# panbanda/islands

Measured on AMD Instinct MI355X. Metric: queries/sec @ recall@10>=0.95, 10Mx768 ef=128, higher is better.
Workload: dtype f32; 1 GPU; 10000000 x 768 f32 rows resident in HBM (in-memory provider), hierarchical Gaussian mixture, graph by the harness (tools/synth.py::build_graph: k-means medoid levels flattened into one layer, diversified links, parent->child and reverse edges), deg<= 60 (mean 38.6), query batch 1024, k=10, ef=128, cosine; nodes=10000000, dim=768, query_batch=1024, k=10, ef=128, graph=harness, distinct_leaves=False, parallelism=single, searches_in_flight=32, distinct_batches=497, replayed_queries=1688

## Files before the change

### include/islands_amd.h

```cpp
#ifndef ISLANDS_AMD_H
#define ISLANDS_AMD_H

#include <stddef.h>
#include <stdint.h>

#ifdef __cplusplus
extern "C" {
#endif

#define ISL_ABI_VERSION 3

typedef int32_t isl_status;

enum {
  ISL_OK = 0,
  ISL_ERR_DIMENSION_MISMATCH = 1,
  ISL_ERR_EMPTY_COLLECTION = 2,
  ISL_ERR_INVALID_CONFIG = 3,
  ISL_ERR_INDEX_NOT_BUILT = 4,
  ISL_ERR_NODE_NOT_FOUND = 5,
  ISL_ERR_SERIALIZATION = 6,
  ISL_ERR_DESERIALIZATION = 7,
  ISL_ERR_IO = 8,
  ISL_ERR_HNSW = 9,
// ... 150 lines not shown
                                  uint64_t k, uint64_t ef, uint64_t* out_ids, float* out_dist,
                                  uint32_t* out_count, uint64_t* token);
isl_status isl_search_batch_device(const isl_index* idx, const float* d_queries, uint64_t nq,
                                   uint64_t d, uint64_t k, uint64_t ef, uint64_t* d_out_ids,
                                   float* d_out_dist, uint32_t* d_out_count, void* stream);
isl_status isl_search_batch_device_async(const isl_index* idx, const float* d_queries, uint64_t nq,
                                         uint64_t d, uint64_t k, uint64_t ef, uint64_t* d_out_ids,
                                         float* d_out_dist, uint32_t* d_out_count, void* stream,
                                         uint64_t* token);
isl_status isl_search_wait_stats(const isl_index* idx, uint64_t token, isl_search_stats* stats);
isl_status isl_search_wait(const isl_index* idx, uint64_t token);
isl_status isl_search_stream_wait(const isl_index* idx, uint64_t token, void* stream);
isl_status isl_index_group_counters(const isl_index* idx, uint64_t* launches, uint64_t* shared_launches,
                                    uint64_t* shared_calls);
isl_status isl_index_group_markers(const isl_index* idx, uint64_t* calls, uint64_t* marked_calls);
isl_status isl_search(const isl_index* idx, const float* query, uint64_t d, uint64_t k,
                      uint64_t* out_ids, float* out_dist, uint32_t* out_count);

isl_status isl_search_last_stats(const isl_index* idx, isl_search_stats* out);

#define ISL_MAX_ENTRY_SEEDS 65536ull
isl_status isl_index_select_entry_seeds(isl_index* idx, uint64_t count, uint64_t* out_ids, uint64_t* out_count);
isl_status isl_index_set_entry_seeds(isl_index* idx, const uint64_t* ids, uint64_t count);
isl_status isl_index_entry_seeds(const isl_index* idx, uint64_t* out, uint64_t cap, uint64_t* count);
isl_status isl_index_pick_entries(const isl_index* idx, const float* queries, uint64_t nq, uint64_t d,
                                  uint64_t* out_ids, int32_t mem, void* stream);

isl_status isl_distance(int32_t metric, const float* a, uint64_t na, const float* b, uint64_t nb,
                        float* out);
isl_status isl_distance_squared(int32_t metric, const float* a, uint64_t na, const float* b,
// ... 192 lines not shown
```

### include/islands_amd.hpp

```cpp
#pragma once

#include <cstdint>
#include <optional>
#include <stdexcept>
#include <string>
#include <utility>
#include <vector>

#include "islands_amd.h"

namespace islands::core {

struct CoreError : std::runtime_error {
  isl_status status;
  uint64_t expected, actual, node;
  CoreError(isl_status s, const std::string& msg, uint64_t e = 0, uint64_t a = 0, uint64_t n = 0)
      : std::runtime_error(msg), status(s), expected(e), actual(a), node(n) {}
  std::string kind() const { return isl_status_name(status); }
};

inline void check(isl_status s) {
  if (s != ISL_OK)
    throw CoreError(s, isl_last_error_message(), isl_last_error_expected(),
                    isl_last_error_actual(), isl_last_error_node());
// ... 222 lines not shown
    return out;
  }
  void attach_pq_codes(const isl_pq* pq, const std::vector<uint16_t>& codes, uint64_t n) {
    check(isl_index_set_pq_codes(h_, pq, codes.data(), n, ISL_MEM_HOST));
  }
  std::vector<std::pair<uint64_t, float>> search_two_level(const std::vector<float>& query, uint64_t k,
                                                           uint64_t ef, float rerank_ratio) const {
    std::vector<uint64_t> ids(k ? k : 1);
    std::vector<float> dist(k ? k : 1);
    uint32_t cnt = 0;
    check(isl_search_two_level_batch(h_, query.data(), 1, query.size(), k, ef, rerank_ratio, ids.data(),
                                     dist.data(), &cnt));
    std::vector<std::pair<uint64_t, float>> out;
    for (uint32_t i = 0; i < cnt; i++) out.emplace_back(ids[i], dist[i]);
    return out;
  }
  isl_index* handle() const { return h_; }

 private:
  explicit LeannIndex(std::nullptr_t) {}
  isl_index* h_ = nullptr;
};

struct SearchResult {
  uint64_t id = 0;
  float score = 0.f;
  std::optional<std::vector<float>> vector;
  std::optional<std::string> text;
  float to_similarity() const { return 1.0f / (1.0f + score); }
};
// ... 251 lines not shown
```

### islands_amd/_ffi.py

```python
from __future__ import annotations

import ctypes as C
import os

os.environ.setdefault("GPU_MAX_HW_QUEUES", "32")

_HERE = os.path.dirname(os.path.abspath(__file__))
LIB_PATH = os.environ.get("ISL_AMD_LIB") or os.path.join(_HERE, "lib", "libislands_amd.so")

u64, u32, i32, f32 = C.c_uint64, C.c_uint32, C.c_int32, C.c_float
P = C.POINTER


class LeannConfigC(C.Structure):
    _fields_ = [
        ("m", u64), ("m0", u64), ("ef_construction", u64), ("ml", C.c_double),
        ("max_layers", u64), ("metric", u32), ("ef_search", u64), ("beam_width", u64),
        ("prune_ratio", f32), ("pruning_strategy", u32), ("high_degree_pruning", C.c_uint8),
        ("hub_percentile", f32), ("is_compact", C.c_uint8), ("is_recompute", C.c_uint8),
    ]


class BertConfigC(C.Structure):
    _fields_ = [("vocab_size", u32), ("hidden", u32), ("layers", u32), ("heads", u32),
# ... 67 lines not shown
                                         C.c_void_p, C.c_void_p, C.c_void_p]),
    "isl_search_two_level_batch_device": (i32, [C.c_void_p, C.c_void_p, u64, u64, u64, u64,
                                                C.c_float, C.c_void_p, C.c_void_p, C.c_void_p,
                                                C.c_void_p]),
    "isl_search_two_level_batch_device_async": (i32, [C.c_void_p, C.c_void_p, u64, u64, u64, u64,
                                                      C.c_float, C.c_void_p, C.c_void_p, C.c_void_p,
                                                      C.c_void_p, P(u64)]),
    "isl_search_batch_device": (i32, [C.c_void_p, C.c_void_p, u64, u64, u64, u64, C.c_void_p,
                                      C.c_void_p, C.c_void_p, C.c_void_p]),
    "isl_search_batch_device_async": (i32, [C.c_void_p, C.c_void_p, u64, u64, u64, u64, C.c_void_p,
                                            C.c_void_p, C.c_void_p, C.c_void_p, P(u64)]),
    "isl_search_wait": (i32, [C.c_void_p, u64]),
    "isl_search_stream_wait": (i32, [C.c_void_p, u64, C.c_void_p]),
    "isl_index_group_counters": (i32, [C.c_void_p, P(u64), P(u64), P(u64)]),
    "isl_index_group_markers": (i32, [C.c_void_p, P(u64), P(u64)]),
    "isl_shard_record_bytes": (u64, [u64, u64]),
    "isl_merge_topk_packed_async": (i32, [u64, u64, u64, C.c_void_p, u64, C.c_void_p, u64, C.c_void_p, C.c_void_p,
                                          C.c_void_p, C.c_void_p, C.c_void_p, i32, C.c_void_p]),
    "isl_shard_unique_id": (i32, [C.c_void_p]),
    "isl_shard_group_create": (i32, [i32, i32, i32, C.c_void_p, P(C.c_void_p)]),
    "isl_shard_group_create_host": (i32, [i32, i32, i32, C.c_void_p, C.c_void_p, P(C.c_void_p)]),
    "isl_shard_group_info": (i32, [C.c_void_p, P(i32), P(i32), P(i32), P(i32)]),
    "isl_shard_group_free": (None, [C.c_void_p]),
    "isl_sharded_searcher_new": (i32, [C.c_void_p, C.c_void_p, u64, C.c_void_p, i32, P(C.c_void_p)]),
    "isl_sharded_searcher_free": (None, [C.c_void_p]),
    "isl_sharded_prepare": (i32, [C.c_void_p, u64, u64, u64]),
    "isl_sharded_submit": (i32, [C.c_void_p, C.c_void_p, u64, u64, u64, u64, C.c_void_p, P(u64)]),
    "isl_sharded_result": (i32, [C.c_void_p, u64, P(C.c_void_p), P(C.c_void_p), P(C.c_void_p), P(C.c_void_p),
                                 P(SearchStatsC)]),
    "isl_sharded_search_batch": (i32, [C.c_void_p, C.c_void_p, u64, u64, u64, u64, C.c_void_p, C.c_void_p,
# ... 125 lines not shown
```

### islands_amd/csrc/api_index.hip

```cpp
#include "device_common.hip.h"
#include "encoder.hpp"

#include <algorithm>
#include <cmath>
#include <new>

namespace isl {

ErrorRecord& last_error() {
  thread_local ErrorRecord rec;
  return rec;
}

isl_status fail(isl_status st, const char* fmt, ...) {
  char buf[512];
  va_list ap;
  va_start(ap, fmt);
  vsnprintf(buf, sizeof(buf), fmt, ap);
  va_end(ap);
  last_error().message = buf;
  return st;
}

isl_status fail_dim(uint64_t expected, uint64_t actual) {
// ... 38 lines not shown
    g_devices[device].ncu = prop.multiProcessorCount;
    g_devices[device].state = 1;
  }
  return ISL_OK;
}

int device_cu_count(int32_t device) {
  return (device >= 0 && device < 64 && g_devices[device].state == 1) ? g_devices[device].ncu : 256;
}

void free_workspace(SearchWorkspace& ws) {
  if (ws.ev0) (void)hipEventDestroy(ws.ev0);
  if (ws.ev1) (void)hipEventDestroy(ws.ev1);
  if (ws.ev_in) (void)hipEventDestroy(ws.ev_in);
  if (ws.ev_done) (void)hipEventDestroy(ws.ev_done);
  ws = SearchWorkspace{};
}

}

using namespace isl;

static int g_hw_queues_at_load = 4;
__attribute__((constructor)) static void isl_default_hw_queues() {
  if (const char* e = getenv("GPU_MAX_HW_QUEUES")) {
    const int v = atoi(e);
    if (v > 0) g_hw_queues_at_load = v;
  }
  setenv("GPU_MAX_HW_QUEUES", "32", 0);
}
// ... 754 lines not shown
```

### islands_amd/csrc/common.hpp

```cpp
#pragma once

#include <hip/hip_runtime.h>

#include <algorithm>
#include <cstdarg>
#include <cstdint>
#include <cstdlib>
#include <cstdio>
#include <cstring>
#include <atomic>
#include <chrono>
#include <mutex>
#include <string>
#include <thread>
#include <type_traits>
#include <vector>

#include "../../include/islands_amd.h"
#include "device_buffer.hpp"
#include "row_table.hpp"

namespace isl {

struct ErrorRecord {
// ... 45 lines not shown
  DeviceBuffer<uint32_t> qsel;
  DeviceBuffer<uint32_t> qsel_h;
  DeviceBuffer<uint64_t> plog;
  DeviceBuffer<float> q_stage;
  DeviceBuffer<uint64_t> ids_stage;
  DeviceBuffer<float> dist_stage;
  DeviceBuffer<uint32_t> count_stage;
  PinnedBuffer<float> h_q;
  PinnedBuffer<uint64_t> h_ids;
  PinnedBuffer<float> h_dist;
  PinnedBuffer<uint32_t> h_count;
  hipStream_t stream = nullptr;
  hipEvent_t ev0 = nullptr, ev1 = nullptr, ev_in = nullptr, ev_done = nullptr;
  float launch_ms = 0.0f;
  bool launch_ms_read = false;
  bool busy = false;
  bool waiting = false;
  bool enqueued = false;
  bool ticket_clean = false;
  bool publish_results = false;
  uint64_t token = 0;
  uint64_t nq_inflight = 0, k_inflight = 0;
  uint32_t ef_inflight = 0;
  bool fast_inflight = false;
  hipStream_t st_inflight = nullptr;
  uint64_t* u_ids = nullptr;
  float* u_dist = nullptr;
  uint32_t* u_count = nullptr;
  PinnedBuffer<uint32_t> h_status;
  PinnedBuffer<uint32_t> h_ctr;
// ... 26 lines not shown
  uint64_t alloc_mark = 0;
  isl_search_stats stats{};
  bool grp = false;
  SearchWorkspace* grp_launch = nullptr;
  uint32_t grp_offset = 0;
  hipEvent_t grp_ready = nullptr;
  bool grp_marked = false;
  uint64_t grp_allocs = 0;
  bool grp_failed = false;
  isl_status grp_status = ISL_OK;
  ErrorRecord grp_error;
  int32_t pool_lane = -1;
  bool union_launch = false;
  PinnedBuffer<uint64_t> h_members;
  DeviceBuffer<uint32_t> grp_scratch;
};

constexpr int kSearchLanes = 32;

int hw_queues_at_load();
constexpr int kGroupBelowQueues = 8;
struct GroupSwitches { bool off; uint32_t cap, room; bool mark_always, trace; };
inline GroupSwitches group_switches() {
  auto num = [](const char* name) -> uint32_t {
    const char* e = getenv(name);
    const long long v = e ? atoll(e) : 0;
    return v > 0 ? (uint32_t)std::min<long long>(v, 0x7FFFFFFF) : 0u;
  };
  const char* off = getenv("ISL_NO_GROUP");
  const bool is_off = (off && *off) ? strcmp(off, "0") != 0 : hw_queues_at_load() >= kGroupBelowQueues;
// ... 82 lines not shown

  mutable std::mutex mu;
  mutable std::mutex recompute_mu;
  struct RecJoin {
    std::mutex mu;
    std::mutex leader;
    std::vector<void*> waiting;
  };
  mutable RecJoin rec_join;
  mutable isl::SearchWorkspace ws[isl::kSearchLanes];
  mutable isl::ExactPool pool;
  mutable uint64_t next_token = 1;
  const isl::GroupSwitches group_sw = isl::group_switches();
  mutable std::mutex group_mu;
  mutable isl::GroupState* group = nullptr;
};

struct isl_hnsw {
  isl_index* core = nullptr;
  uint64_t m = 0, m0 = 0, ef_construction = 0;
  uint64_t dim = 0;
  double ml = 0.0;
  uint64_t max_layers = 16;
  int32_t device = 0;
  std::vector<const uint64_t*> layer_off;
  std::vector<const uint32_t*> layer_adj;
  mutable std::mutex host_mu;
  mutable bool host_valid = false;
  mutable std::vector<std::vector<uint64_t>> h_off;
  mutable std::vector<std::vector<uint64_t>> h_adj;
// ... 28 lines not shown
```

### islands_amd/csrc/search.hip

```cpp
#include "search_geometry.hpp"
#include "search_internal.hpp"

#include <cmath>

using namespace isl_lane;

namespace {

__global__ void fill_u32_kernel(uint32_t* p, uint64_t n, uint32_t v) {
  uint64_t i = (uint64_t)blockIdx.x * blockDim.x + threadIdx.x;
  uint64_t stride = (uint64_t)gridDim.x * blockDim.x;
  for (; i < n; i += stride) p[i] = v;
}

struct PublishParams {
  const uint32_t* src[6];
  uint32_t* dst[6];
  uint32_t words[6];
  uint32_t ticket_seg;
};
__global__ void publish_kernel(PublishParams pp) {
  const uint32_t seg = blockIdx.y;
  const uint32_t n = pp.words[seg];
  const uint32_t* __restrict__ src = pp.src[seg];
  uint32_t* __restrict__ dst = pp.dst[seg];
  for (uint32_t i = blockIdx.x * blockDim.x + threadIdx.x; i < n; i += gridDim.x * blockDim.x) {
    dst[i] = src[i];
    if (seg == pp.ticket_seg) const_cast<uint32_t*>(src)[i] = 0u;
  }
}
__global__ void copy_u128_kernel(const uint4* __restrict__ src, uint4* __restrict__ dst, uint64_t n) {
  for (uint64_t i = (uint64_t)blockIdx.x * blockDim.x + threadIdx.x; i < n; i += (uint64_t)gridDim.x * blockDim.x)
    dst[i] = src[i];
}
__global__ void copy_u32_kernel(const uint32_t* __restrict__ src, uint32_t* __restrict__ dst, uint64_t n) {
  for (uint64_t i = (uint64_t)blockIdx.x * blockDim.x + threadIdx.x; i < n; i += (uint64_t)gridDim.x * blockDim.x)
    dst[i] = src[i];
}

__global__ void seed_redo_kernel(const uint32_t* __restrict__ list, uint32_t n, uint32_t* __restrict__ redo,
                                 uint32_t* __restrict__ ticket) {
  for (uint32_t i = threadIdx.x; i < n; i += blockDim.x) redo[i] = list[i];
  if (threadIdx.x == 0) ticket[1] = n;
// ... 22 lines not shown
  return st;
}

}

isl_status isl_lane::ensure_lane_stream(const isl_index* idx, isl::SearchWorkspace& ws) {
  if (ws.stream) return ISL_OK;
  bool created = false;
  hipStream_t st = pool_stream(idx->device, ws.pool_lane >= 0 ? (uint32_t)ws.pool_lane : (uint32_t)(&ws - idx->ws), &created);
  if (!st) return isl::fail(ISL_ERR_DEVICE, "hipStreamCreate failed for a search lane");
  if (created) ws.alloc_events++;
  if (!ws.ev_done) { ISL_HIP(hipEventCreateWithFlags(&ws.ev_done, hipEventDisableTiming)); ws.alloc_events++; }
  if (!ws.ev0) { ISL_HIP(hipEventCreate(&ws.ev0)); ws.alloc_events++; }
  if (!ws.ev1) { ISL_HIP(hipEventCreate(&ws.ev1)); ws.alloc_events++; }
  if (!ws.ev_in) { ISL_HIP(hipEventCreateWithFlags(&ws.ev_in, hipEventDisableTiming)); ws.alloc_events++; }
  if (!ws.ticket) {
    ISL_TRY(ws.ticket.reserve(16, &ws.alloc_events));
    ws.ticket_clean = false;
  }
  ISL_TRY(ws.h_head.reserve(16, &ws.alloc_events));
  ws.stream = st;
  return ISL_OK;
}

void isl_lane::copy_words(const uint32_t* src, uint32_t* dst, uint64_t n, uint32_t grid, uint32_t block, hipStream_t st) {
  hipLaunchKernelGGL(copy_u32_kernel, dim3(grid), dim3(block), 0, st, src, dst, n);
}

isl_status isl_lane::prepare_workspace(const isl_index* idx, isl::SearchWorkspace& ws, uint32_t nq, uint32_t slots,
                                       uint32_t plog_cap) {
// ... 72 lines not shown
}

namespace {

__global__ void pad_rows_kernel(const uint64_t* __restrict__ off, const uint32_t* __restrict__ adj, uint64_t n,
                                uint32_t W, uint32_t* __restrict__ ell, uint32_t* __restrict__ deg) {
  const uint64_t row = (uint64_t)blockIdx.x * 4 + (threadIdx.x >> 6);
  const uint32_t lane = threadIdx.x & 63;
  if (row >= n) return;
  const uint64_t o0 = off[row];
  const uint32_t d = (uint32_t)(off[row + 1] - o0);
  for (uint32_t i = lane; i < W; i += 64) ell[row * W + i] = i < d ? adj[o0 + i] : EMPTY;
  if (lane == 0) deg[row] = d;
}

isl_status publish(isl::SearchWorkspace& ws, uint64_t nq, uint64_t k, hipStream_t st) {
  PublishParams pp{};
  uint32_t n = 0;
  auto seg = [&](const void* src, void* dst, uint64_t words) {
    pp.src[n] = (const uint32_t*)src; pp.dst[n] = (uint32_t*)dst; pp.words[n] = (uint32_t)words; ++n;
  };
  seg(ws.status, ws.h_status, nq);
  seg(ws.ctr, ws.h_ctr, nq * 4);
  pp.ticket_seg = n;
  seg(ws.ticket, ws.h_head, 16);
  if (ws.publish_results) {
    seg(ws.count_stage, ws.h_count, nq);
    if (k) {
      seg(ws.ids_stage, ws.h_ids, nq * k * 2);
      seg(ws.dist_stage, ws.h_dist, nq * k);
    }
  }
  hipLaunchKernelGGL(publish_kernel, dim3(16, n), dim3(256), 0, st, pp);
  ISL_HIP(hipGetLastError());
  ws.ticket_clean = true;
  return ISL_OK;
}


void launch_fast(const isl_launch::FastKernel& k, uint32_t grid, size_t lds, hipStream_t st, const SearchParams& p) {
  switch (k.S) {
    case 1: isl_launch::launch_fast_segments<1>(k, grid, lds, st, &p); break;
    case 2: isl_launch::launch_fast_segments<2>(k, grid, lds, st, &p); break;
    case 4: isl_launch::launch_fast_segments<4>(k, grid, lds, st, &p); break;
    default: isl_launch::launch_fast_segments<8>(k, grid, lds, st, &p); break;
  }
}

isl_status search_enqueue_impl(const isl_index* idx, isl::SearchWorkspace& ws, const SearchCall& c,
                               const RoundPlan& plan, bool warm) {
  const uint64_t nq = c.nq, d = c.d, k = c.k;
  if (nq > 0x7FFFFFFFull) return isl::fail(ISL_ERR_INVALID_ARGUMENT, "too many queries");
// ... 203 lines not shown
      launch_fast(fk, grid, cg.fg.lds, st, p);
      p.qsel_mode = 0;
    } else if (!skip_fast) {
      launch_fast(fk, grid, cg.fg.lds, st, p);
    }
    ISL_HIP(hipGetLastError());
    p.nq = (uint32_t)nq;
  } else if (!warm && !resume) {
    std::vector<uint32_t> all(nq);
    for (uint64_t i = 0; i < nq; i++) all[i] = (uint32_t)i;
    uint32_t head0[4] = {0, (uint32_t)nq, 0, 0};
    ISL_HIP(hipMemcpyAsync(ws.redo, all.data(), nq * 4, hipMemcpyHostToDevice, st));
    ISL_HIP(hipMemcpyAsync(ws.ticket, head0, 16, hipMemcpyHostToDevice, st));
    ISL_HIP(hipStreamSynchronize(st));
  }
  if (!tl) {
    uint32_t grid = (uint32_t)std::min<uint64_t>(nq_grid, idx->pool.slots);
    isl_launch::launch_exact(metric, idx->is_hnsw, grid, cg.exact_lds, st, &p);
    ISL_HIP(hipGetLastError());
  }
  ISL_HIP(hipEventRecord(ws.ev1, st));
  ws.st_inflight = st;
  if (warm) return ISL_OK;

  if (!ws.union_launch) {
    ISL_TRY(publish(ws, nq, k, st));
    ISL_HIP(hipEventRecord(ws.ev_done, st));
  }
  ws.enqueued = true;
  ws.nq_inflight = nq;
  ws.k_inflight = k;
  ws.ef_inflight = ef;
  ws.fast_inflight = use_fast;
  return ISL_OK;
}

struct LastStats { const isl_index* idx = nullptr; isl_search_stats st{}; };
thread_local LastStats tl_last_stats;
void note_last_stats(const isl_index* idx, const isl_search_stats& st) {
  tl_last_stats.idx = idx;
  tl_last_stats.st = st;
}

}

isl_status isl_lane::search_enqueue(const isl_index* idx, isl::SearchWorkspace& ws, const SearchCall& c,
                                      const RoundPlan& plan, bool warm) {
  const isl_status st = search_enqueue_impl(idx, ws, c, plan, warm);
  if (st != ISL_OK) {
    const isl::ErrorRecord keep = isl::last_error();
    hipStream_t s = call_stream(ws, c);
    if (c.mode == StreamMode::USER || s) (void)hipStreamSynchronize(s);
    (void)hipGetLastError();
    ws.ticket_clean = false;
    ws.enqueued = false;
    isl::last_error() = keep;
  }
  return st;
}

isl_status isl_lane::search_finish(const isl_index* idx, isl::SearchWorkspace& ws, uint32_t* misses,
                                     bool defer_statuses) {
  if (!ws.enqueued) return isl::fail(ISL_ERR_INVALID_ARGUMENT, "no search in flight for this token");
  ws.enqueued = false;
  const uint64_t nq = ws.nq_inflight;
  const bool use_fast = ws.fast_inflight;
  isl::SearchWorkspace& lw = ws.grp_launch ? *ws.grp_launch : ws;
  ISL_HIP(hipEventSynchronize(lw.ev_done));
  const uint32_t* status = ws.h_status;
  const uint32_t* ctr = ws.h_ctr;
  const uint32_t* head = ws.h_head;
  isl::DeviceBuffer<uint64_t> d_prof = std::move(ws.d_prof);
  float ms = 0.0f;
  {
    static std::mutex ms_mu;
    std::lock_guard<std::mutex> lock(ms_mu);
    if (!lw.launch_ms_read) {
      (void)hipEventElapsedTime(&lw.launch_ms, lw.ev0, lw.ev1);
      lw.launch_ms_read = true;
    }
    ms = lw.launch_ms;
  }

  isl_search_stats& ss = ws.stats;
  ss = isl_search_stats{};
  ss.queries = nq;
  ss.exact_path = head[1];
  ss.replayed = head[3];
  ss.kernel_ms = ms;
  ss.allocations = ws.alloc_events - ws.alloc_mark + ws.grp_allocs;
  for (uint64_t i = 0; i < nq; i++) {
    ss.expansions += ctr[i * 4 + 0];
    ss.edges += ctr[i * 4 + 1];
// ... 546 lines not shown
  }
  if (st == ISL_OK && ws->u_count) host_copy_out(*ws, ws->nq_inflight, ws->k_inflight, ws->u_ids, ws->u_dist, ws->u_count);
  if (stats) *stats = ws->stats;
  note_last_stats(idx, ws->stats);
  return st;
}

isl_status isl_search_wait(const isl_index* idx, uint64_t token) { return isl_search_wait_stats(idx, token, nullptr); }

isl_status isl_search_stream_wait(const isl_index* idx, uint64_t token, void* stream) {
  if (!idx) return isl::fail(ISL_ERR_INVALID_ARGUMENT, "index is NULL");
  if (token == 0) return ISL_OK;
  ISL_TRY(isl::use_device(idx->device));
  isl::SearchWorkspace* found = nullptr;
  isl::SearchWorkspace* grouped = nullptr;
  {
    std::lock_guard<std::mutex> lock(idx->mu);
    for (auto& w : idx->ws)
      if (w.busy && w.token == token) {
        if (w.grp) { grouped = &w; break; }
        if (!w.threaded) {
          ISL_HIP(hipStreamWaitEvent((hipStream_t)stream, w.ev1, 0));
          return ISL_OK;
        }
        if (!w.worker) return ISL_OK;
        if (w.waiting) return isl::fail(ISL_ERR_INVALID_ARGUMENT, "the call is being waited for on another thread");
        found = &w;
        w.waiting = true;
        break;
      }
  }
  if (grouped) {
    if (group_before_wait(idx, *grouped) == ISL_OK) ISL_HIP(hipStreamWaitEvent((hipStream_t)stream, grouped->grp_ready, 0));
    return ISL_OK;
  }
  if (!found) return isl::fail(ISL_ERR_INVALID_ARGUMENT, "unknown or already completed search token");
  found->worker->join();
  delete found->worker;
  found->worker = nullptr;
  {
    std::lock_guard<std::mutex> lock(idx->mu);
    found->waiting = false;
  }
  return ISL_OK;
}

static isl_status search_batch_host(const isl_index* idx, SearchCall c) {
  uint64_t* const out_ids = c.ids;
// ... 70 lines not shown
isl_status isl_search_two_level_batch_device_async(const isl_index* idx, const float* d_queries, uint64_t nq,
                                                   uint64_t d, uint64_t k, uint64_t ef, float rerank_ratio,
                                                   uint64_t* d_out_ids, float* d_out_dist, uint32_t* d_out_count,
                                                   void* stream, uint64_t* token) {
  return search_batch_device_async(idx, SearchCall{d_queries, nq, d, k, ef, d_out_ids, d_out_dist, d_out_count,
                                                   (hipStream_t)stream, StreamMode::USER, true, rerank_ratio}, token);
}

isl_status isl_search(const isl_index* idx, const float* query, uint64_t d, uint64_t k,
                      uint64_t* out_ids, float* out_dist, uint32_t* out_count) {
  if (!idx) return isl::fail(ISL_ERR_INVALID_ARGUMENT, "index is NULL");
  return isl_search_batch(idx, query, 1, d, k, idx->cfg.ef_search, out_ids, out_dist,
                          out_count);
}

isl_status isl_search_last_stats(const isl_index* idx, isl_search_stats* out) {
  if (!idx || !out) return isl::fail(ISL_ERR_INVALID_ARGUMENT, "NULL argument");
  *out = tl_last_stats.idx == idx ? tl_last_stats.st : isl_search_stats{};
  return ISL_OK;
}

}
```

### islands_amd/csrc/search_group.hip

```cpp
#include <cstdarg>
#include <ctime>
#include <memory>

#include "search_geometry.hpp"
#include "search_group_plan.hpp"
#include "search_internal.hpp"

using namespace isl_lane;

namespace isl {

struct GroupState {
  isl_group::Planner plan;
  std::vector<std::unique_ptr<SearchWorkspace>> slots;
  SearchCall calls[kSearchLanes];
  uint64_t launches = 0, shared_launches = 0, shared_calls = 0;
  uint64_t arrived_calls = 0, marked_calls = 0;
  uint32_t launch_of[kSearchLanes] = {};
};

}

namespace {

// ... 29 lines not shown
}

struct ScatterParams {
  const GroupMember* tab;
  const uint64_t* ids;
  const float* dist;
  const uint32_t* count;
  const uint32_t* status;
  const uint32_t* ctr;
  const uint32_t* redo;
  const uint2* plog;
  uint32_t* ticket;
  uint32_t* h_head;
  uint32_t* scratch;
  uint32_t k, ef, plog_cap;
};

__device__ __forceinline__ uint32_t wave_sum(uint32_t v) {
  for (int o = 32; o > 0; o >>= 1) v += (uint32_t)__shfl_xor((int)v, o);
  return v;
}

__global__ void group_scatter_kernel(ScatterParams sp) {
  const GroupMember m = sp.tab[blockIdx.y];
  const uint32_t lane = threadIdx.x & 63;
  const uint32_t wave = blockIdx.x * (blockDim.x >> 6) + (threadIdx.x >> 6);
  const uint32_t nwaves = gridDim.x * (blockDim.x >> 6);
  const uint32_t k = sp.k;
  const uint32_t nredo = *((volatile uint32_t*)&sp.ticket[1]);
  uint32_t n_exact = 0, n_replayed = 0;
  for (uint32_t qi = wave; qi < m.nq; qi += nwaves) {
    const uint32_t q = m.offset + qi;
    const uint32_t cnt = sp.count[q];
    const uint32_t st = sp.status[q];
    if (lane == 0) {
      m.count[qi] = cnt;
      m.h_status[qi] = st;
    }
    if (lane < 4) m.h_ctr[qi * 4 + lane] = sp.ctr[q * 4 + lane];
    const uint32_t outn = cnt < k ? cnt : k;
    for (uint32_t e = lane; e < outn; e += 64) {
      m.ids[(uint64_t)qi * k + e] = sp.ids[(uint64_t)q * k + e];
      m.dist[(uint64_t)qi * k + e] = sp.dist[(uint64_t)q * k + e];
    }
    bool hit = false;
    for (uint32_t i = lane; i < nredo; i += 64) hit |= sp.redo[i] == q;
    if (__ballot(hit)) { n_exact += 1; continue; }
    if (st != QS_OK || outn == 0) continue;
    const uint32_t* db = reinterpret_cast<const uint32_t*>(sp.dist) + (uint64_t)q * k;
    bool dup = false;
    for (uint32_t e = lane; e + 1 < outn; e += 64) dup |= db[e] == db[e + 1];
    bool tie = __ballot(dup) != 0;
    const uint32_t pushes = sp.ctr[q * 4 + 3];
    const uint32_t len = pushes < sp.ef ? pushes : sp.ef;
    if (!tie && outn == k && len >= k + 1) {
      const uint32_t dk = db[k - 1];
      uint32_t returned = 0, pushed = 0;
      for (uint32_t e = lane; e < k; e += 64) returned += db[e] == dk;
      const uint2* pl = sp.plog + (uint64_t)q * sp.plog_cap;
      const uint32_t logged = pushes < sp.plog_cap ? pushes : sp.plog_cap;
      for (uint32_t i = lane; i < logged; i += 64) pushed += pl[i].x == dk;
      tie = wave_sum(pushed) > wave_sum(returned);
// ... 5 lines not shown
    if (n_exact) atomicAdd(&mine[0], n_exact);
    if (n_replayed) atomicAdd(&mine[1], n_replayed);
  }
  __threadfence();
  __syncthreads();
  if (threadIdx.x != 0) return;
  if (atomicAdd(&mine[2], 1u) == gridDim.x - 1) {
    __threadfence();
    const uint32_t ex = atomicExch(&mine[0], 0u), rp = atomicExch(&mine[1], 0u);
    mine[2] = 0u;
    for (uint32_t i = 0; i < 16; ++i) m.h_head[i] = i == 1 ? ex : i == 3 ? rp : 0u;
  }
  uint32_t* all = sp.scratch + kMaxMembers * 4;
  if (atomicAdd(all, 1u) == gridDim.x * gridDim.y - 1) {
    *all = 0u;
    for (uint32_t i = 0; i < 16; ++i) {
      sp.h_head[i] = sp.ticket[i];
      sp.ticket[i] = 0u;
    }
  }
}

__global__ void zero_u32_kernel(uint32_t* p, uint32_t n) {
  for (uint32_t i = blockIdx.x * blockDim.x + threadIdx.x; i < n; i += gridDim.x * blockDim.x) p[i] = 0u;
}

void trace_line(const char* fmt, ...) {
  timespec b{}, m{};
  clock_gettime(CLOCK_BOOTTIME, &b);
  clock_gettime(CLOCK_MONOTONIC, &m);
  char text[512];
  va_list ap;
  va_start(ap, fmt);
// ... 42 lines not shown
void grow_slots(const isl_index* idx, isl::GroupState& g, uint32_t n) {
  if (g.slots.size() < n) g.slots.resize(n);
  g.plan.configure(group_cap(idx), n);
}

isl_status enqueue_alone(const isl_index* idx, isl::GroupState& g, const isl_group::Launch& L) {
  const uint32_t lane_no = L.members[0].call;
  isl::SearchWorkspace& ws = idx->ws[lane_no];
  SearchCall c = g.calls[lane_no];
  c.user_stream = nullptr;
  c.mode = ws.grp_marked ? StreamMode::OWN_AFTER_EVENT : StreamMode::OWN;
  ISL_TRY(search_enqueue(idx, ws, c));
  ws.grp_launch = nullptr;
  ws.grp_offset = 0;
  ws.grp_ready = ws.ev1;
  return ISL_OK;
}

isl_status enqueue_group_impl(const isl_index* idx, isl::GroupState& g, const isl_group::Launch& L,
                              isl::SearchWorkspace& gw) {
  const uint64_t d = L.key.d, k = L.key.k;
  const uint32_t nm = (uint32_t)L.members.size();
  if (nm > kMaxMembers) return isl::fail(ISL_ERR_SEARCH, "Search error: %u calls in one group launch", nm);
  CallGeometry cg;
  ISL_TRY(call_geometry(idx, d, k, L.key.ef, nullptr, cg));
  ISL_TRY(prepare_slot(idx, gw, L.nq, d, k));
  ISL_TRY(prepare_workspace(idx, gw, L.nq, (uint32_t)std::min<uint64_t>(L.nq, cg.lane_slots), cg.plog_cap));
  GroupMember* tab = reinterpret_cast<GroupMember*>(gw.h_members.get());
  for (uint32_t i = 0; i < nm; ++i) {
    const isl_group::Member& mb = L.members[i];
// ... 5 lines not shown
    if (ws.grp_marked) ISL_HIP(hipStreamWaitEvent(gw.stream, ws.ev_in, 0));
  }
  hipLaunchKernelGGL(group_gather_kernel, dim3(64, nm), dim3(256), 0, gw.stream, tab, gw.q_stage.get(), (uint32_t)d);
  ISL_HIP(hipGetLastError());
  SearchCall u;
  u.queries = gw.q_stage;
  u.nq = L.nq;
  u.d = d;
  u.k = k;
  u.ef = L.key.ef;
  u.ids = gw.ids_stage;
  u.dist = gw.dist_stage;
  u.count = gw.count_stage;
  u.mode = StreamMode::OWN;
  ISL_TRY(search_enqueue(idx, gw, u));
  ScatterParams sp{};
  sp.tab = tab;
  sp.ids = gw.ids_stage;
  sp.dist = gw.dist_stage;
  sp.count = gw.count_stage;
  sp.status = gw.status;
  sp.ctr = gw.ctr;
  sp.redo = gw.redo;
  sp.plog = reinterpret_cast<const uint2*>(gw.plog.get());
  sp.ticket = gw.ticket;
  sp.h_head = gw.h_head;
  sp.scratch = gw.grp_scratch;
  sp.k = (uint32_t)k;
  sp.ef = cg.ef;
  sp.plog_cap = cg.plog_cap;
  hipLaunchKernelGGL(group_scatter_kernel, dim3(kScatterBlocks, nm), dim3(256), 0, gw.stream, sp);
  ISL_HIP(hipGetLastError());
  gw.ticket_clean = true;
  ISL_HIP(hipEventRecord(gw.ev_done, gw.stream));
  return ISL_OK;
}

isl_status enqueue_group(const isl_index* idx, isl::GroupState& g, const isl_group::Launch& L) {
  isl::SearchWorkspace& gw = slot(g, L.workspace);
  const uint64_t mark = gw.alloc_events;
  const isl_status st = enqueue_group_impl(idx, g, L, gw);
  gw.enqueued = false;
  if (st != ISL_OK) {
    const isl::ErrorRecord keep = isl::last_error();
    if (gw.stream) (void)hipStreamSynchronize(gw.stream);
    (void)hipGetLastError();
    gw.ticket_clean = false;
    isl::last_error() = keep;
// ... 109 lines not shown
  ws.grp_failed = false;
  ws.grp_launch = nullptr;
  ws.grp_allocs = 0;
  poll(idx, g);
  const uint32_t room = idx->group_sw.room ? idx->group_sw.room : cg.slots;
  g.plan.arrive(lane_no, (uint32_t)c.nq, isl_group::Key{c.d, c.k, cg.ef}, room);
  submit(idx, g, isl_group::kNone);
  if (ws.grp_failed) {
    ws.grp = false;
    isl::last_error() = ws.grp_error;
    return ws.grp_status;
  }
  return ISL_OK;
}

void isl_lane::group_pump(const isl_index* idx) {
  std::lock_guard<std::mutex> lock(idx->group_mu);
  if (!idx->group || !idx->group->plan.any_held()) return;
  poll(idx, *idx->group);
  submit(idx, *idx->group, isl_group::kNone);
}

isl_status isl_lane::group_before_wait(const isl_index* idx, isl::SearchWorkspace& ws) {
  std::lock_guard<std::mutex> lock(idx->group_mu);
  isl::GroupState& g = state_of(idx);
  poll(idx, g);
  submit(idx, g, (uint32_t)(&ws - idx->ws));
  if (ws.grp_failed) {
    isl::last_error() = ws.grp_error;
    return ws.grp_status;
// ... 32 lines not shown
    ISL_TRY(prepare_workspace(idx, gw, (uint32_t)nq, (uint32_t)std::min<uint64_t>(nq, ovf_waves), plog_cap));
    if (idx->seeds.count()) ISL_TRY(gw.q_entry.reserve(nq * 4, &gw.alloc_events));
  }
  for (int round = 0; round < 2; ++round) {
    for (uint32_t w = 0; w < n; ++w) {
      isl::SearchWorkspace& gw = *g.slots[w];
      GroupMember* tab = reinterpret_cast<GroupMember*>(gw.h_members.get());
      tab[0] = GroupMember{};
      hipLaunchKernelGGL(group_gather_kernel, dim3(1, 1), dim3(256), 0, gw.stream, tab, gw.q_stage.get(), (uint32_t)d);
      ISL_HIP(hipGetLastError());
      SearchCall warm_call;
      warm_call.d = d;
      warm_call.k = std::min<uint64_t>(max_k, max_ef);
      warm_call.ef = max_ef;
      ISL_TRY(search_enqueue(idx, gw, warm_call, RoundPlan{}, true));
      ScatterParams sp{};
      sp.tab = tab;
      sp.ids = gw.ids_stage;
      sp.dist = gw.dist_stage;
      sp.count = gw.count_stage;
      sp.status = gw.status;
      sp.ctr = gw.ctr;
      sp.redo = gw.redo;
      sp.plog = reinterpret_cast<const uint2*>(gw.plog.get());
      sp.ticket = gw.ticket;
      sp.h_head = gw.h_head;
      sp.scratch = gw.grp_scratch;
      sp.k = (uint32_t)std::max<uint64_t>(max_k, 1);
      sp.ef = (uint32_t)max_ef;
      sp.plog_cap = plog_cap;
      tab[0].h_head = gw.h_head;
      hipLaunchKernelGGL(group_scatter_kernel, dim3(kScatterBlocks, 1), dim3(256), 0, gw.stream, sp);
      ISL_HIP(hipGetLastError());
      gw.ticket_clean = true;
      ISL_HIP(hipEventRecord(gw.ev_done, gw.stream));
    }
    for (uint32_t w = 0; w < n; ++w) ISL_HIP(hipStreamSynchronize(g.slots[w]->stream));
  }
  return ISL_OK;
}

extern "C" isl_status isl_index_group_counters(const isl_index* idx, uint64_t* launches, uint64_t* shared_launches,
                                               uint64_t* shared_calls) {
  if (!idx) return isl::fail(ISL_ERR_INVALID_ARGUMENT, "index is NULL");
  std::lock_guard<std::mutex> lock(idx->group_mu);
  const isl::GroupState* g = idx->group;
  if (launches) *launches = g ? g->launches : 0;
  if (shared_launches) *shared_launches = g ? g->shared_launches : 0;
// ... 29 lines not shown
```

### islands_amd/csrc/search_internal.hpp

```cpp
#pragma once

#include "common.hpp"

namespace isl_lane __attribute__((visibility("hidden"))) {

enum class StreamMode { OWN, USER, OWN_AFTER_USER, OWN_AFTER_EVENT };

struct SearchCall {
  const float* queries = nullptr;
  uint64_t nq = 0, d = 0, k = 0, ef = 0;
  uint64_t* ids = nullptr;
  float* dist = nullptr;
  uint32_t* count = nullptr;
  hipStream_t user_stream = nullptr;
  StreamMode mode = StreamMode::OWN;
  bool two_level = false;
  float ratio = 0.0f;
};
inline hipStream_t call_stream(const isl::SearchWorkspace& ws, const SearchCall& c) {
  return c.mode == StreamMode::USER ? c.user_stream : ws.stream;
}

struct RoundPlan {
  uint32_t active = 0;
// ... 4 lines not shown
  uint32_t retry = 0;
  uint32_t window_scale = 1;
  bool tables_built = false;
};

isl_status ensure_lane_stream(const isl_index* idx, isl::SearchWorkspace& ws);
isl_status ensure_pool(const isl_index* idx, isl::SearchWorkspace& ws);
void copy_words(const uint32_t* src, uint32_t* dst, uint64_t n, uint32_t grid, uint32_t block, hipStream_t st);
isl_status prepare_workspace(const isl_index* idx, isl::SearchWorkspace& ws, uint32_t nq, uint32_t slots,
                             uint32_t plog_cap);
isl_status search_enqueue(const isl_index* idx, isl::SearchWorkspace& ws, const SearchCall& c,
                          const RoundPlan& plan = RoundPlan{}, bool warm = false);
isl_status search_finish(const isl_index* idx, isl::SearchWorkspace& ws, uint32_t* misses = nullptr,
                         bool defer_statuses = false);
isl_status search_statuses(isl::SearchWorkspace& ws, uint64_t nq);
isl_status search_sync(const isl_index* idx, isl::SearchWorkspace& ws, const SearchCall& c);

isl_status prepare_recompute(isl::SearchWorkspace& ws, uint64_t nq, uint64_t state_words_per_query);
isl_status tl_retry_short(isl::SearchWorkspace& ws, uint64_t nq, uint32_t& window_scale, uint32_t* nshort);
isl_status recompute_rounds(const isl_index* idx, isl::SearchWorkspace& ws, const SearchCall& c);
isl_status recompute_coalesced(const isl_index* idx, isl::SearchWorkspace& ws, const SearchCall& c);

bool group_takes(const isl_index* idx, const SearchCall& c);
isl_status group_arrive(const isl_index* idx, isl::SearchWorkspace& ws, const SearchCall& c);
void group_pump(const isl_index* idx);
isl_status group_before_wait(const isl_index* idx, isl::SearchWorkspace& ws);
void group_after_wait(const isl_index* idx, isl::SearchWorkspace& ws);
isl_status group_prepare(const isl_index* idx, uint64_t max_nq, uint64_t max_ef, uint64_t max_k, int32_t lanes,
                         uint32_t ovf_waves, uint32_t plog_cap);

}
```

Baseline: 1.664 million queries/s.

## Defer exact redo round to wait time and skip it when no queries need it

Instead of always launching the exact-recompute (redo) kernel in-stream after the fast search, the launch parameters are saved and the redo is issued at wait time only if the device head counter shows pending redo queries. Publish and group-scatter kernels gain a phase argument so phase 1 keeps the ticket when redo is pending and phase 2 republishes the results. This removes a kernel launch and its stream time when no queries overflow. The cost is a host round-trip and extra serialization when redo is needed, plus more complex wait paths.

```diff
diff --git a/include/islands_amd.h b/include/islands_amd.h
--- a/include/islands_amd.h
+++ b/include/islands_amd.h
@@ -188,6 +188,7 @@
 isl_status isl_index_group_counters(const isl_index* idx, uint64_t* launches, uint64_t* shared_launches,
                                     uint64_t* shared_calls);
 isl_status isl_index_group_markers(const isl_index* idx, uint64_t* calls, uint64_t* marked_calls);
+isl_status isl_index_redo_rounds(const isl_index* idx, uint64_t out[2]);
 isl_status isl_search(const isl_index* idx, const float* query, uint64_t d, uint64_t k,
                       uint64_t* out_ids, float* out_dist, uint32_t* out_count);
 
diff --git a/include/islands_amd.hpp b/include/islands_amd.hpp
--- a/include/islands_amd.hpp
+++ b/include/islands_amd.hpp
@@ -260,6 +260,11 @@
     std::vector<std::pair<uint64_t, float>> out;
     for (uint32_t i = 0; i < cnt; i++) out.emplace_back(ids[i], dist[i]);
     return out;
+  }
+  std::pair<uint64_t, uint64_t> redo_rounds() const {
+    uint64_t out[2] = {0, 0};
+    check(isl_index_redo_rounds(h_, out));
+    return {out[0], out[1]};
   }
   isl_index* handle() const { return h_; }
 
diff --git a/islands_amd/_ffi.py b/islands_amd/_ffi.py
--- a/islands_amd/_ffi.py
+++ b/islands_amd/_ffi.py
@@ -105,6 +105,7 @@
     "isl_search_stream_wait": (i32, [C.c_void_p, u64, C.c_void_p]),
     "isl_index_group_counters": (i32, [C.c_void_p, P(u64), P(u64), P(u64)]),
     "isl_index_group_markers": (i32, [C.c_void_p, P(u64), P(u64)]),
+    "isl_index_redo_rounds": (i32, [C.c_void_p, P(u64)]),
     "isl_shard_record_bytes": (u64, [u64, u64]),
     "isl_merge_topk_packed_async": (i32, [u64, u64, u64, C.c_void_p, u64, C.c_void_p, u64, C.c_void_p, C.c_void_p,
                                           C.c_void_p, C.c_void_p, C.c_void_p, i32, C.c_void_p]),
diff --git a/islands_amd/csrc/api_index.hip b/islands_amd/csrc/api_index.hip
--- a/islands_amd/csrc/api_index.hip
+++ b/islands_amd/csrc/api_index.hip
@@ -76,6 +76,9 @@
   if (ws.ev1) (void)hipEventDestroy(ws.ev1);
   if (ws.ev_in) (void)hipEventDestroy(ws.ev_in);
   if (ws.ev_done) (void)hipEventDestroy(ws.ev_done);
+  if (ws.ev_r0) (void)hipEventDestroy(ws.ev_r0);
+  if (ws.ev_r1) (void)hipEventDestroy(ws.ev_r1);
+  if (ws.ev_done2) (void)hipEventDestroy(ws.ev_done2);
   ws = SearchWorkspace{};
 }
 
diff --git a/islands_amd/csrc/common.hpp b/islands_amd/csrc/common.hpp
--- a/islands_amd/csrc/common.hpp
+++ b/islands_amd/csrc/common.hpp
@@ -83,6 +83,10 @@
   hipEvent_t ev0 = nullptr, ev1 = nullptr, ev_in = nullptr, ev_done = nullptr;
   float launch_ms = 0.0f;
   bool launch_ms_read = false;
+  hipEvent_t ev_r0 = nullptr, ev_r1 = nullptr, ev_done2 = nullptr;
+  bool redo_deferred = false;
+  bool redo_phase2 = false;
+  std::vector<unsigned char> redo_call;
   bool busy = false;
   bool waiting = false;
   bool enqueued = false;
@@ -139,6 +143,7 @@
   bool union_launch = false;
   PinnedBuffer<uint64_t> h_members;
   DeviceBuffer<uint32_t> grp_scratch;
+  uint32_t grp_members = 0, grp_plog_cap = 0;
 };
 
 constexpr int kSearchLanes = 32;
@@ -251,6 +256,7 @@
   const isl::GroupSwitches group_sw = isl::group_switches();
   mutable std::mutex group_mu;
   mutable isl::GroupState* group = nullptr;
+  mutable std::atomic<uint64_t> redo_instream{0}, redo_rounds{0};
 };
 
 struct isl_hnsw {
diff --git a/islands_amd/csrc/search.hip b/islands_amd/csrc/search.hip
--- a/islands_amd/csrc/search.hip
+++ b/islands_amd/csrc/search.hip
@@ -1,5 +1,6 @@
 #include "search_geometry.hpp"
 #include "search_internal.hpp"
+#include "search_redo_plan.hpp"
 
 #include <cmath>
 
@@ -18,15 +19,20 @@
   uint32_t* dst[6];
   uint32_t words[6];
   uint32_t ticket_seg;
+  uint32_t phase;
 };
 __global__ void publish_kernel(PublishParams pp) {
   const uint32_t seg = blockIdx.y;
   const uint32_t n = pp.words[seg];
-  const uint32_t* __restrict__ src = pp.src[seg];
-  uint32_t* __restrict__ dst = pp.dst[seg];
+  const uint32_t* src = pp.src[seg];
+  uint32_t* dst = pp.dst[seg];
+  const bool heads = seg == pp.ticket_seg;
+  const bool pending = heads && *((const volatile uint32_t*)&src[1]) != 0u;
+  if (heads && pp.phase == 2u && !pending) return;
+  const bool keep = pp.phase == 1u && pending;
   for (uint32_t i = blockIdx.x * blockDim.x + threadIdx.x; i < n; i += gridDim.x * blockDim.x) {
     dst[i] = src[i];
-    if (seg == pp.ticket_seg) const_cast<uint32_t*>(src)[i] = 0u;
+    if (heads && !keep) const_cast<uint32_t*>(src)[i] = 0u;
   }
 }
 __global__ void copy_u128_kernel(const uint4* __restrict__ src, uint4* __restrict__ dst, uint64_t n) {
@@ -79,6 +85,9 @@
   if (!ws.ev0) { ISL_HIP(hipEventCreate(&ws.ev0)); ws.alloc_events++; }
   if (!ws.ev1) { ISL_HIP(hipEventCreate(&ws.ev1)); ws.alloc_events++; }
   if (!ws.ev_in) { ISL_HIP(hipEventCreateWithFlags(&ws.ev_in, hipEventDisableTiming)); ws.alloc_events++; }
+  if (!ws.ev_r0) { ISL_HIP(hipEventCreate(&ws.ev_r0)); ws.alloc_events++; }
+  if (!ws.ev_r1) { ISL_HIP(hipEventCreate(&ws.ev_r1)); ws.alloc_events++; }
+  if (!ws.ev_done2) { ISL_HIP(hipEventCreateWithFlags(&ws.ev_done2, hipEventDisableTiming)); ws.alloc_events++; }
   if (!ws.ticket) {
     ISL_TRY(ws.ticket.reserve(16, &ws.alloc_events));
     ws.ticket_clean = false;
@@ -181,8 +190,9 @@
   if (lane == 0) deg[row] = d;
 }
 
-isl_status publish(isl::SearchWorkspace& ws, uint64_t nq, uint64_t k, hipStream_t st) {
+isl_status publish(isl::SearchWorkspace& ws, uint64_t nq, uint64_t k, hipStream_t st, uint32_t phase = 0) {
   PublishParams pp{};
+  pp.phase = phase;
   uint32_t n = 0;
   auto seg = [&](const void* src, void* dst, uint64_t words) {
     pp.src[n] = (const uint32_t*)src; pp.dst[n] = (uint32_t*)dst; pp.words[n] = (uint32_t)words; ++n;
@@ -200,9 +210,16 @@
   }
   hipLaunchKernelGGL(publish_kernel, dim3(16, n), dim3(256), 0, st, pp);
   ISL_HIP(hipGetLastError());
-  ws.ticket_clean = true;
-  return ISL_OK;
-}
+  ws.ticket_clean = phase != 1;
+  return ISL_OK;
+}
+
+struct RedoCall {
+  SearchParams p;
+  uint32_t grid;
+  size_t lds;
+  uint64_t nq, k;
+};
 
 
 void launch_fast(const isl_launch::FastKernel& k, uint32_t grid, size_t lds, hipStream_t st, const SearchParams& p) {
@@ -436,17 +453,36 @@
     ISL_HIP(hipMemcpyAsync(ws.ticket, head0, 16, hipMemcpyHostToDevice, st));
     ISL_HIP(hipStreamSynchronize(st));
   }
+  isl_redo::Call rc;
+  rc.use_fast = use_fast;
+  rc.in_memory = !idx->recompute;
+  rc.resume = resume;
+  rc.two_level = tl != nullptr;
+  rc.warm = warm;
+  rc.caller_stream = c.mode == StreamMode::USER;
+  const char* instream_env = getenv("ISL_REDO_INSTREAM");
+  rc.instream_switch = instream_env && *instream_env && strcmp(instream_env, "0") != 0;
+  ws.redo_deferred = false;
+  ws.redo_phase2 = false;
   if (!tl) {
     uint32_t grid = (uint32_t)std::min<uint64_t>(nq_grid, idx->pool.slots);
-    isl_launch::launch_exact(metric, idx->is_hnsw, grid, cg.exact_lds, st, &p);
-    ISL_HIP(hipGetLastError());
+    if (isl_redo::decide(isl_redo::When::Enqueue, rc, isl_redo::State{}) == isl_redo::Action::Deferred) {
+      RedoCall keep{p, grid, cg.exact_lds, nq, k};
+      ws.redo_call.resize(sizeof keep);
+      memcpy(ws.redo_call.data(), &keep, sizeof keep);
+      ws.redo_deferred = true;
+    } else {
+      isl_launch::launch_exact(metric, idx->is_hnsw, grid, cg.exact_lds, st, &p);
+      ISL_HIP(hipGetLastError());
+      if (!warm) idx->redo_instream.fetch_add(1, std::memory_order_relaxed);
+    }
   }
   ISL_HIP(hipEventRecord(ws.ev1, st));
   ws.st_inflight = st;
   if (warm) return ISL_OK;
 
   if (!ws.union_launch) {
-    ISL_TRY(publish(ws, nq, k, st));
+    ISL_TRY(publish(ws, nq, k, st, ws.redo_deferred ? 1u : 0u));
     ISL_HIP(hipEventRecord(ws.ev_done, st));
   }
   ws.enqueued = true;
@@ -476,9 +512,45 @@
     (void)hipGetLastError();
     ws.ticket_clean = false;
     ws.enqueued = false;
+    ws.redo_deferred = false;
     isl::last_error() = keep;
   }
   return st;
+}
+
+isl_status isl_lane::redo_at_wait(const isl_index* idx, isl::SearchWorkspace& lw, bool stream_wait, bool* phase2) {
+  std::lock_guard<std::mutex> lock(idx->group_mu);
+  isl_redo::State s;
+  s.deferred = lw.redo_deferred;
+  s.phase2_enqueued = lw.redo_phase2;
+  if (s.deferred && !s.phase2_enqueued) {
+    bool complete = !stream_wait;
+    if (stream_wait) {
+      complete = hipEventQuery(lw.ev_done) == hipSuccess;
+      if (!complete) (void)hipGetLastError();
+    }
+    if (complete) s.count = lw.h_head[1] ? isl_redo::Count::NonZero : isl_redo::Count::Zero;
+  }
+  const isl_redo::When when = stream_wait ? isl_redo::When::StreamWait : isl_redo::When::HostWait;
+  if (isl_redo::decide(when, isl_redo::Call{}, s) == isl_redo::Action::Phase2Now) {
+    if (lw.redo_call.size() != sizeof(RedoCall)) return isl::fail(ISL_ERR_SEARCH, "Search error: no redo round kept for the launch");
+    RedoCall rc;
+    memcpy(&rc, lw.redo_call.data(), sizeof rc);
+    hipStream_t st = lw.st_inflight;
+    ISL_HIP(hipEventRecord(lw.ev_r0, st));
+    isl_launch::launch_exact((int)idx->cfg.metric, idx->is_hnsw, rc.grid, rc.lds, st, &rc.p);
+    ISL_HIP(hipGetLastError());
+    ISL_HIP(hipEventRecord(lw.ev_r1, st));
+    if (lw.union_launch) ISL_TRY(group_scatter_again(idx, lw));
+    else ISL_TRY(publish(lw, rc.nq, rc.k, st, 2u));
+    ISL_HIP(hipEventRecord(lw.ev_done2, st));
+    lw.redo_phase2 = true;
+    idx->redo_rounds.fetch_add(1, std::memory_order_relaxed);
+  } else if (s.deferred && s.count == isl_redo::Count::Zero) {
+    lw.ticket_clean = true;
+  }
+  *phase2 = lw.redo_phase2;
+  return ISL_OK;
 }
 
 isl_status isl_lane::search_finish(const isl_index* idx, isl::SearchWorkspace& ws, uint32_t* misses,
@@ -489,6 +561,9 @@
   const bool use_fast = ws.fast_inflight;
   isl::SearchWorkspace& lw = ws.grp_launch ? *ws.grp_launch : ws;
   ISL_HIP(hipEventSynchronize(lw.ev_done));
+  bool phase2 = false;
+  ISL_TRY(redo_at_wait(idx, lw, false, &phase2));
+  if (phase2) ISL_HIP(hipEventSynchronize(lw.ev_done2));
   const uint32_t* status = ws.h_status;
   const uint32_t* ctr = ws.h_ctr;
   const uint32_t* head = ws.h_head;
@@ -499,6 +574,11 @@
     std::lock_guard<std::mutex> lock(ms_mu);
     if (!lw.launch_ms_read) {
       (void)hipEventElapsedTime(&lw.launch_ms, lw.ev0, lw.ev1);
+      if (phase2) {
+        float redo_ms = 0.0f;
+        (void)hipEventElapsedTime(&redo_ms, lw.ev_r0, lw.ev_r1);
+        lw.launch_ms += redo_ms;
+      }
       lw.launch_ms_read = true;
     }
     ms = lw.launch_ms;
@@ -1075,15 +1155,13 @@
   ISL_TRY(isl::use_device(idx->device));
   isl::SearchWorkspace* found = nullptr;
   isl::SearchWorkspace* grouped = nullptr;
+  isl::SearchWorkspace* plain = nullptr;
   {
     std::lock_guard<std::mutex> lock(idx->mu);
     for (auto& w : idx->ws)
       if (w.busy && w.token == token) {
         if (w.grp) { grouped = &w; break; }
-        if (!w.threaded) {
-          ISL_HIP(hipStreamWaitEvent((hipStream_t)stream, w.ev1, 0));
-          return ISL_OK;
-        }
+        if (!w.threaded) { plain = &w; break; }
         if (!w.worker) return ISL_OK;
         if (w.waiting) return isl::fail(ISL_ERR_INVALID_ARGUMENT, "the call is being waited for on another thread");
         found = &w;
@@ -1091,8 +1169,19 @@
         break;
       }
   }
+  if (plain) {
+    bool phase2 = false;
+    ISL_TRY(redo_at_wait(idx, *plain, true, &phase2));
+    ISL_HIP(hipStreamWaitEvent((hipStream_t)stream, phase2 ? plain->ev_done2 : plain->ev1, 0));
+    return ISL_OK;
+  }
   if (grouped) {
-    if (group_before_wait(idx, *grouped) == ISL_OK) ISL_HIP(hipStreamWaitEvent((hipStream_t)stream, grouped->grp_ready, 0));
+    if (group_before_wait(idx, *grouped) == ISL_OK) {
+      isl::SearchWorkspace& lw = grouped->grp_launch ? *grouped->grp_launch : *grouped;
+      bool phase2 = false;
+      ISL_TRY(redo_at_wait(idx, lw, true, &phase2));
+      ISL_HIP(hipStreamWaitEvent((hipStream_t)stream, phase2 ? lw.ev_done2 : grouped->grp_ready, 0));
+    }
     return ISL_OK;
   }
   if (!found) return isl::fail(ISL_ERR_INVALID_ARGUMENT, "unknown or already completed search token");
@@ -1193,6 +1282,13 @@
                           out_count);
 }
 
+isl_status isl_index_redo_rounds(const isl_index* idx, uint64_t out[2]) {
+  if (!idx || !out) return isl::fail(ISL_ERR_INVALID_ARGUMENT, "NULL argument");
+  out[0] = idx->redo_instream.load(std::memory_order_relaxed);
+  out[1] = idx->redo_rounds.load(std::memory_order_relaxed);
+  return ISL_OK;
+}
+
 isl_status isl_search_last_stats(const isl_index* idx, isl_search_stats* out) {
   if (!idx || !out) return isl::fail(ISL_ERR_INVALID_ARGUMENT, "NULL argument");
   *out = tl_last_stats.idx == idx ? tl_last_stats.st : isl_search_stats{};
diff --git a/islands_amd/csrc/search_group.hip b/islands_amd/csrc/search_group.hip
--- a/islands_amd/csrc/search_group.hip
+++ b/islands_amd/csrc/search_group.hip
@@ -67,6 +67,7 @@
   uint32_t* h_head;
   uint32_t* scratch;
   uint32_t k, ef, plog_cap;
+  uint32_t phase;
 };
 
 __device__ __forceinline__ uint32_t wave_sum(uint32_t v) {
@@ -84,6 +85,10 @@
   uint32_t n_exact = 0, n_replayed = 0;
   for (uint32_t qi = wave; qi < m.nq; qi += nwaves) {
     const uint32_t q = m.offset + qi;
+    bool hit = false;
+    for (uint32_t i = lane; i < nredo; i += 64) hit |= sp.redo[i] == q;
+    const bool redone = __ballot(hit) != 0;
+    if (redone && sp.phase == 1u) { n_exact += 1; continue; }
     const uint32_t cnt = sp.count[q];
     const uint32_t st = sp.status[q];
     if (lane == 0) {
@@ -96,9 +101,7 @@
       m.ids[(uint64_t)qi * k + e] = sp.ids[(uint64_t)q * k + e];
       m.dist[(uint64_t)qi * k + e] = sp.dist[(uint64_t)q * k + e];
     }
-    bool hit = false;
-    for (uint32_t i = lane; i < nredo; i += 64) hit |= sp.redo[i] == q;
-    if (__ballot(hit)) { n_exact += 1; continue; }
+    if (redone) { n_exact += 1; continue; }
     if (st != QS_OK || outn == 0) continue;
     const uint32_t* db = reinterpret_cast<const uint32_t*>(sp.dist) + (uint64_t)q * k;
     bool dup = false;
@@ -134,9 +137,11 @@
   uint32_t* all = sp.scratch + kMaxMembers * 4;
   if (atomicAdd(all, 1u) == gridDim.x * gridDim.y - 1) {
     *all = 0u;
+    const bool pending = nredo != 0u;
+    if (sp.phase == 2u && !pending) return;
     for (uint32_t i = 0; i < 16; ++i) {
       sp.h_head[i] = sp.ticket[i];
-      sp.ticket[i] = 0u;
+      if (!(sp.phase == 1u && pending)) sp.ticket[i] = 0u;
     }
   }
 }
@@ -209,6 +214,28 @@
   ws.grp_launch = nullptr;
   ws.grp_offset = 0;
   ws.grp_ready = ws.ev1;
+  return ISL_OK;
+}
+
+isl_status scatter(isl::SearchWorkspace& gw, uint32_t nm, uint32_t k, uint32_t ef, uint32_t plog_cap, uint32_t phase) {
+  ScatterParams sp{};
+  sp.tab = reinterpret_cast<const GroupMember*>(gw.h_members.get());
+  sp.ids = gw.ids_stage;
+  sp.dist = gw.dist_stage;
+  sp.count = gw.count_stage;
+  sp.status = gw.status;
+  sp.ctr = gw.ctr;
+  sp.redo = gw.redo;
+  sp.plog = reinterpret_cast<const uint2*>(gw.plog.get());
+  sp.ticket = gw.ticket;
+  sp.h_head = gw.h_head;
+  sp.scratch = gw.grp_scratch;
+  sp.k = k;
+  sp.ef = ef;
+  sp.plog_cap = plog_cap;
+  sp.phase = phase;
+  hipLaunchKernelGGL(group_scatter_kernel, dim3(kScatterBlocks, nm), dim3(256), 0, gw.stream, sp);
+  ISL_HIP(hipGetLastError());
   return ISL_OK;
 }
 
@@ -244,24 +271,10 @@
   u.count = gw.count_stage;
   u.mode = StreamMode::OWN;
   ISL_TRY(search_enqueue(idx, gw, u));
-  ScatterParams sp{};
-  sp.tab = tab;
-  sp.ids = gw.ids_stage;
-  sp.dist = gw.dist_stage;
-  sp.count = gw.count_stage;
-  sp.status = gw.status;
-  sp.ctr = gw.ctr;
-  sp.redo = gw.redo;
-  sp.plog = reinterpret_cast<const uint2*>(gw.plog.get());
-  sp.ticket = gw.ticket;
-  sp.h_head = gw.h_head;
-  sp.scratch = gw.grp_scratch;
-  sp.k = (uint32_t)k;
-  sp.ef = cg.ef;
-  sp.plog_cap = cg.plog_cap;
-  hipLaunchKernelGGL(group_scatter_kernel, dim3(kScatterBlocks, nm), dim3(256), 0, gw.stream, sp);
-  ISL_HIP(hipGetLastError());
-  gw.ticket_clean = true;
+  gw.grp_members = nm;
+  gw.grp_plog_cap = cg.plog_cap;
+  ISL_TRY(scatter(gw, nm, (uint32_t)k, cg.ef, cg.plog_cap, gw.redo_deferred ? 1u : 0u));
+  gw.ticket_clean = !gw.redo_deferred;
   ISL_HIP(hipEventRecord(gw.ev_done, gw.stream));
   return ISL_OK;
 }
@@ -401,6 +414,13 @@
   return ISL_OK;
 }
 
+isl_status isl_lane::group_scatter_again(const isl_index* idx, isl::SearchWorkspace& gw) {
+  (void)idx;
+  ISL_TRY(scatter(gw, gw.grp_members, (uint32_t)gw.k_inflight, gw.ef_inflight, gw.grp_plog_cap, 2u));
+  gw.ticket_clean = true;
+  return ISL_OK;
+}
+
 void isl_lane::group_pump(const isl_index* idx) {
   std::lock_guard<std::mutex> lock(idx->group_mu);
   if (!idx->group || !idx->group->plan.any_held()) return;
@@ -463,24 +483,8 @@
       warm_call.k = std::min<uint64_t>(max_k, max_ef);
       warm_call.ef = max_ef;
       ISL_TRY(search_enqueue(idx, gw, warm_call, RoundPlan{}, true));
-      ScatterParams sp{};
-      sp.tab = tab;
-      sp.ids = gw.ids_stage;
-      sp.dist = gw.dist_stage;
-      sp.count = gw.count_stage;
-      sp.status = gw.status;
-      sp.ctr = gw.ctr;
-      sp.redo = gw.redo;
-      sp.plog = reinterpret_cast<const uint2*>(gw.plog.get());
-      sp.ticket = gw.ticket;
-      sp.h_head = gw.h_head;
-      sp.scratch = gw.grp_scratch;
-      sp.k = (uint32_t)std::max<uint64_t>(max_k, 1);
-      sp.ef = (uint32_t)max_ef;
-      sp.plog_cap = plog_cap;
       tab[0].h_head = gw.h_head;
-      hipLaunchKernelGGL(group_scatter_kernel, dim3(kScatterBlocks, 1), dim3(256), 0, gw.stream, sp);
-      ISL_HIP(hipGetLastError());
+      ISL_TRY(scatter(gw, 1, (uint32_t)std::max<uint64_t>(max_k, 1), (uint32_t)max_ef, plog_cap, 0u));
       gw.ticket_clean = true;
       ISL_HIP(hipEventRecord(gw.ev_done, gw.stream));
     }
diff --git a/islands_amd/csrc/search_internal.hpp b/islands_amd/csrc/search_internal.hpp
--- a/islands_amd/csrc/search_internal.hpp
+++ b/islands_amd/csrc/search_internal.hpp
@@ -42,6 +42,7 @@
 isl_status search_finish(const isl_index* idx, isl::SearchWorkspace& ws, uint32_t* misses = nullptr,
                          bool defer_statuses = false);
 isl_status search_statuses(isl::SearchWorkspace& ws, uint64_t nq);
+isl_status redo_at_wait(const isl_index* idx, isl::SearchWorkspace& lw, bool stream_wait, bool* phase2);
 isl_status search_sync(const isl_index* idx, isl::SearchWorkspace& ws, const SearchCall& c);
 
 isl_status prepare_recompute(isl::SearchWorkspace& ws, uint64_t nq, uint64_t state_words_per_query);
@@ -54,6 +55,7 @@
 void group_pump(const isl_index* idx);
 isl_status group_before_wait(const isl_index* idx, isl::SearchWorkspace& ws);
 void group_after_wait(const isl_index* idx, isl::SearchWorkspace& ws);
+isl_status group_scatter_again(const isl_index* idx, isl::SearchWorkspace& gw);
 isl_status group_prepare(const isl_index* idx, uint64_t max_nq, uint64_t max_ef, uint64_t max_k, int32_t lanes,
                          uint32_t ovf_waves, uint32_t plog_cap);
 
diff --git a/islands_amd/csrc/search_redo_plan.hpp b/islands_amd/csrc/search_redo_plan.hpp
--- /dev/null
+++ b/islands_amd/csrc/search_redo_plan.hpp
@@ -0,0 +1,56 @@
+#pragma once
+
+#include <cstdint>
+
+namespace isl_redo {
+
+enum class When : uint8_t {
+  Enqueue,
+  HostWait,
+  StreamWait,
+};
+enum class Count : uint8_t { Unknown, Zero, NonZero };
+enum class Action : uint8_t {
+  InStream,
+  Deferred,
+  Phase2Now,
+  Done,
+};
+
+struct Call {
+  bool use_fast = false;
+  bool in_memory = true;
+  bool resume = false;
+  bool two_level = false;
+  bool warm = false;
+  bool caller_stream = false;
+  bool instream_switch = false;
+};
+
+struct State {
+  bool deferred = false;
+  bool phase2_enqueued = false;
+  Count count = Count::Unknown;
+};
+
+inline bool deferrable(const Call& c) {
+  return c.use_fast && c.in_memory && !c.resume && !c.two_level && !c.warm && !c.caller_stream && !c.instream_switch;
+}
+
+inline Action decide(When when, const Call& c, const State& s) {
+  if (when == When::Enqueue) return deferrable(c) ? Action::Deferred : Action::InStream;
+  if (!s.deferred || s.phase2_enqueued) return Action::Done;
+  if (s.count == Count::Zero) return Action::Done;
+  return Action::Phase2Now;
+}
+
+inline const char* name(Action a) {
+  switch (a) {
+    case Action::InStream: return "in-stream";
+    case Action::Deferred: return "deferred";
+    case Action::Phase2Now: return "phase2";
+    default: return "done";
+  }
+}
+
+}
```

Measured after the change: 1.669 million queries/s, median of 6. No clear change (+0.3%).
